# chg60/phamclust

Measured on AMD Instinct MI355X. Metric: genome-pairs/sec, higher is better.
Workload: dtype int32; 1 GPU; synth(5000,5000) -m peq: full N x N distance-matrix fill; `value` = fills with the genomes resident in HBM and the matrix left in HBM (upload and D2H excluded: see value_wall); n_genomes=5000, n_phams=5000, metric_selector=peq, genome_pairs=12497500, n_genes=531832, n_residues=111773410, parallelism=static pair shard over 1 GPU(s)

## Files before the change

### phamclust_amd/csrc/pc_align.hip

```cpp
#include <numeric>

#include "pc_host.h"

static int small_launch_min() {
    static const int v = [] { const char* e = getenv("PC_SMALL_LAUNCH_MIN"); const int x = e ? atoi(e) : 0; return x > 0 ? x : 192; }();
    return v;
}
static int run_align_classes(pc_ctx* c, const PcTask* task_list, const uint32_t* task_begin , const int32_t* cls_max_lb,
                             uint2* res, hipStream_t st, pc_stats* stats, int ppos) {
    const int nbase = c->ncls_all;
    struct Launch { uint32_t begin, end; int base, mode, max_lb; };
    std::vector<Launch> launches;
    for (int b = 0; b < nbase; ++b) {
        const uint32_t* tb = task_begin + (size_t)b * PC_WAVE_MODES;
        if (tb[PC_WAVE_MODES] == tb[0]) continue;
        const uint32_t n0 = tb[1] - tb[0], n1 = tb[2] - tb[1], n2 = tb[3] - tb[2];
        const int bv = pc_class_variant(b);
        const uint32_t least = (bv >= 0 && pc_nw_variant_w(bv) >= 32) ? 1u : (uint32_t)small_launch_min();
        const bool own2 = n2 >= least, own1 = n1 + (own2 ? 0u : n2) >= least;
        uint32_t at = tb[0];
        const int max_lb = cls_max_lb[b * PC_WAVE_MODES];
        auto put = [&](uint32_t n, int mode) { if (n) launches.push_back({at, at + n, b, mode, max_lb}); at += n; };
        if (own1) { put(n0, PC_MODE_CLASS); put(n1 + (own2 ? 0u : n2), n1 ? PC_MODE_TWO_WAVES : PC_MODE_ONE_WAVE); }
        else put(n0 + n1 + (own2 ? 0u : n2), n0 ? PC_MODE_CLASS : n1 ? PC_MODE_TWO_WAVES : PC_MODE_ONE_WAVE);
// ... 544 lines not shown
        local.n_chunks = 1;
        *stats = local;
    }
    return PC_OK;
}

extern "C" int pc_reduce_dev(pc_ctx* c, int metric, int as_distance, const void* res_dev, void* out_condensed_dev, void* stream) {
    if (!c || !c->uploaded || !c->plan.valid) { pc_set_error("pc_reduce_dev: pc_plan_dev first"); return PC_ERR_STATE; }
    if (!c->plan.whole) { pc_set_error("pc_reduce_dev: the plan in the context is not a whole-matrix plan of an unsharded context (pc_plan_dev)"); return PC_ERR_STATE; }
    if (metric == PC_AAI_PPOS) metric = PC_AAI;
    if (metric != PC_AAI && metric != PC_PEQ) { pc_set_error("pc_reduce_dev: metric %d", metric); return PC_ERR_ARG; }
    if (!out_condensed_dev || (!res_dev && c->plan.n_distinct > 0)) { pc_set_error("pc_reduce_dev: NULL argument"); return PC_ERR_ARG; }
    PC_ON_DEVICE(c);
    hipStream_t st = (hipStream_t)stream;
    int rc = wait_last_work(c, st, true); if (rc != PC_OK) return rc;
    rc = stage_reduce(c, metric, as_distance, (const uint2*)res_dev, (double*)out_condensed_dev, st);
    int rc2 = mark_work(c, st);
    return rc != PC_OK ? abi_rc(rc) : rc2;
}

extern "C" int pc_align_pairs(pc_ctx* c, const int32_t* a_gene, const int32_t* b_gene, int64_t n, int variant,
                              int32_t* n_ident, int32_t* n_diag) {
    if (!c || !c->uploaded) { pc_set_error("pc_align_pairs: upload first"); return PC_ERR_STATE; }
    if (n < 0 || (n > 0 && (!a_gene || !b_gene || !n_ident || !n_diag))) { pc_set_error("pc_align_pairs: NULL argument"); return PC_ERR_ARG; }
    if (n == 0) return PC_OK;
    if (n >= 0x7fffffffLL) { pc_set_error("pc_align_pairs: too many pairs"); return PC_ERR_LIMIT; }
    if (!c->residues_ready) { pc_set_error("pc_align_pairs: the residues are not on the device (pc_upload_residues)"); return PC_ERR_STATE; }
    PC_ON_DEVICE(c);
    int rc = wait_last_work(c, nullptr, false); if (rc != PC_OK) return rc;
    c->plan.valid = false;
    const int G = c->dev.G;
    const int nvar = pc_nw_num_variants();
    int forced = -2;
    if (variant < 0) forced = -1;
    else if (variant > 0) {
        for (int v = 0; v < nvar; ++v) if (pc_nw_variant_w(v) == variant) forced = v;
        if (forced == -2) { pc_set_error("pc_align_pairs: no systolic variant with %d columns per lane", variant); return PC_ERR_ARG; }
    }
    std::vector<int> cls(n);
    std::vector<int32_t> sums(n);
    for (int64_t k = 0; k < n; ++k) {
        if (a_gene[k] < 0 || a_gene[k] >= G || b_gene[k] < 0 || b_gene[k] >= G) { pc_set_error("pc_align_pairs: gene index out of range at %lld", (long long)k); return PC_ERR_ARG; }
        const int la = c->h_gene_len[a_gene[k]], lb = c->h_gene_len[b_gene[k]];
        if (la == 0 || lb == 0) { pc_set_error("pc_align_pairs: empty translation at %lld", (long long)k); return PC_ERR_DATA; }
        int v = forced == -2 ? pc_nw_choose_variant(lb) : forced;
        if (v >= 0 && lb > 64 * pc_nw_variant_w(v) && pc_nw_variant_w(v) < 32) { pc_set_error("pc_align_pairs: column gene of %d residues does not fit variant w=%d (strip-mined passes exist for w = 32, 48, 64)", lb, pc_nw_variant_w(v)); return PC_ERR_ARG; }
        cls[k] = pc_class_of(lb, v, c->h_gene_odd[b_gene[k]] != 0);
        sums[k] = la + lb;
    }
    std::vector<int64_t> order(n);
    std::iota(order.begin(), order.end(), 0);
    std::sort(order.begin(), order.end(), [&](int64_t x, int64_t y) {
        if (cls[x] != cls[y]) return cls[x] < cls[y];
        if (b_gene[x] != b_gene[y]) return b_gene[x] < b_gene[y];
        return x < y;
    });
    std::vector<int32_t> rows(n); std::vector<uint32_t> dest(n); std::vector<PcTask> tasks;
    const int nlc = pc_num_classes() * PC_WAVE_MODES;
    std::vector<uint32_t> cls_task_begin(nlc + 1, 0);
    std::vector<int> cls_maxlb(nlc, 0);
    {
        for (int64_t i = 0; i < n;) {
            const int64_t k = order[i];
            int64_t j = i;
            while (j < n && cls[order[j]] == cls[k] && b_gene[order[j]] == b_gene[k]) ++j;
            const int lb = c->h_gene_len[b_gene[k]];
            const bool odd = c->h_gene_odd[b_gene[k]] != 0;
            const PcBucketCut cut = pc_bucket_cut(lb, j - i, cls[k], odd, forced == -2);
            const int per = cut.per, rem_cls = cut.rem_base;
            const int64_t jmain = i + cut.n_main;
            auto put = [&](int64_t r0, int64_t r1, int base) {
                PcTask t; t.gene = b_gene[k]; t.begin = (int32_t)r0; t.end = (int32_t)r1;
                t.pad = pc_task_launch_class(lb, (int)(r1 - r0), base, forced == -2);
                cls_maxlb[t.pad] = std::max(cls_maxlb[t.pad], lb);
                tasks.push_back(t);
            };
            for (int64_t r = i; r < jmain; r += per) put(r, std::min<int64_t>(jmain, r + per), cls[k]);
            if (rem_cls >= 0) put(jmain, j, rem_cls);
            for (int64_t r = i; r < j; ++r) { rows[r] = a_gene[order[r]]; dest[r] = (uint32_t)order[r]; }
            i = j;
        }
        std::stable_sort(tasks.begin(), tasks.end(), [&](const PcTask& x, const PcTask& y) {
            if (x.pad != y.pad) return x.pad < y.pad;
            const int64_t wx = (int64_t)(x.end - x.begin) * c->h_gene_len[x.gene], wy = (int64_t)(y.end - y.begin) * c->h_gene_len[y.gene];
            return wx > wy;
        });
        size_t at = 0;
        for (int lc = 0; lc <= nlc; ++lc) { while (at < tasks.size() && tasks[at].pad < lc) ++at; cls_task_begin[lc] = (uint32_t)at; }
    }
    DevBuf d_sums, d_ident, d_diag;
    hipStream_t st = c->stream;
    if ((rc = upload_vec(c->b_bucket_row, rows)) || (rc = upload_vec(c->b_bucket_dest, dest)) || (rc = upload_vec(c->b_tasks, tasks)) ||
        (rc = c->b_res.ensure(n * 8)) || (rc = upload_vec(d_sums, sums)) || (rc = d_ident.ensure(n * 4)) || (rc = d_diag.ensure(n * 4))) return abi_rc(rc);
    (void)hipEventRecord(c->ev[1], st);
    for (int lc = 0; lc < nlc; ++lc) {
        const int nt = (int)(cls_task_begin[lc + 1] - cls_task_begin[lc]);
        if (nt <= 0) continue;
        void* scratch = nullptr; size_t sbytes = 0;
        const int base = lc / PC_WAVE_MODES, v = pc_class_variant(base);
        if (v < 0 || pc_launch_is_strip(v, cls_maxlb[lc], lc % PC_WAVE_MODES, 0)) {
            sbytes = v < 0 ? pc_nw_fallback_scratch_bytes(cls_maxlb[lc]) : pc_nw_strip_scratch_bytes(c->max_gene_len, c->n_cu);
            if ((rc = c->b_scratch.ensure(sbytes))) return abi_rc(rc);
            scratch = c->b_scratch.p; sbytes = c->b_scratch.cap;
        }
        rc = pc_launch_nw(v, c->dev, c->b_tasks.as<PcTask>() + cls_task_begin[lc], nt, c->b_bucket_row.as<int32_t>(),
                          c->b_bucket_dest.as<uint32_t>(), c->b_res.as<uint2>(), scratch, sbytes, cls_maxlb[lc], 0, c->tie_rule, pc_class_compare_only(base), st,
// ... 15 lines not shown
```

### phamclust_amd/csrc/pc_nw.hip

```cpp
#include "pc_nw_systolic.h"


struct PcCell { int Ho, E, F; uint32_t SH, SE, SF; };

__device__ __forceinline__ PcCell pc_cell(int Hol, int El, uint32_t SHl, uint32_t SEl, int Hou, int Fu, uint32_t SHu,
                                          uint32_t SFu, int Hod, uint32_t SHd, int sp, bool eq, int rule) {
    PcCell c;
    const int Ee = El - PC_EXT, Fe = Fu - PC_EXT;
    c.E = max(Hol, Ee);
    c.SE = ((rule & 2) ? Hol >= Ee : Hol > Ee) ? SHl : SEl;
    c.F = max(Hou, Fe);
    c.SF = ((rule & 4) ? Hou >= Fe : Hou > Fe) ? SHu : SFu;
    const int D = Hod + sp;
    const int H = max(max(D, c.E), c.F);
    const uint32_t SD = SHd + 0x10000u + (eq ? 1u : 0u);
    const uint32_t ST = (rule & 1) ? ((H == c.E) ? c.SE : c.SF) : ((H == c.F) ? c.SF : c.SE);
    c.SH = (H == D) ? SD : ST;
    c.Ho = H - PC_OPEN;
    return c;
}

__global__ __launch_bounds__(64) void k_nw_general(PcDev d, const PcTask* __restrict__ tasks, int ntasks,
                                                   const int32_t* __restrict__ bucket_row,
                                                   const uint32_t* __restrict__ bucket_dest, uint2* __restrict__ res,
                                                   int4* __restrict__ scratch, int64_t scratch_stride, int ppos, int rule) {
    __shared__ int8_t tab[24][24];
    for (int i = threadIdx.x; i < 576; i += 64) tab[i / 24][i % 24] = (int8_t)(c_b62[i / 24][i % 24] + PC_OPEN);
    __syncthreads();
    int4* sc = scratch + (int64_t)blockIdx.x * scratch_stride;
    const int lane = threadIdx.x;
    for (int task = blockIdx.x; task < ntasks; task += gridDim.x) {
        const PcTask tk = tasks[task];
        const int lb = d.gene_len[tk.gene];
// ... 48 lines not shown

static const int g_variant_w[] = {2, 3, 4, 5, 6, 7, 8, 9, 10, 11, 12, 13, 14, 15, 16, 17, 18, 19, 20, 22, 24, 32, 48, 64};
static const int g_num_variants = (int)(sizeof(g_variant_w) / sizeof(int));

static bool class_inc16(int W, int G);
int pc_nw_num_variants() { return g_num_variants; }
int pc_nw_variant_w(int v) { return (v >= 0 && v < g_num_variants) ? g_variant_w[v] : 0; }
int pc_nw_variant_takes_any_byte(int v) { return v < 0 || v >= g_num_variants || g_variant_w[v] > PC_INC16_MAX_W; }

static bool strip_enabled() { static const bool off = getenv("PC_STRIP") && !atoi(getenv("PC_STRIP")); return !off; }
int pc_nw_launch_is_strip(int variant, int max_lb, int wave_mode, int ppos) {
    if (variant < 0 || variant >= g_num_variants) return 0;
    const int W = g_variant_w[variant];
    if (max_lb > 64 * W) return 1;
    return (!ppos && W >= 32 && wave_mode != PC_MODE_CLASS && strip_enabled()) ? 1 : 0;
}
int pc_nw_strip_passes(int lb, int variant) {
    if (variant < 0 || variant >= g_num_variants || lb <= 0) return 0;
    const int cols = 64 * g_variant_w[variant];
    return (lb + cols - 1) / cols;
}
static int choose_strip_variant(int lb) {
    if (!strip_enabled()) return -1;
    int best = -1; double best_cost = 0;
    for (int v = 0; v < g_num_variants; ++v) {
        const int W = g_variant_w[v];
        if (W < 32) continue;
        const double pen = W >= 64 ? 1.15 : W >= 48 ? 1.08 : 1.04;
        const double cost = (double)pc_nw_strip_passes(lb, v) * (W + 1.0) * pen;
        if (best < 0 || cost < best_cost) { best = v; best_cost = cost; }
    }
    return best;
}
int pc_nw_choose_variant(int lb) {
    if (lb <= 0) return -1;
    if (lb > 64 * PC_MAX_W) return choose_strip_variant(lb);
    int best = -1; double best_cost = 0;
    for (int v = 0; v < g_num_variants; ++v) {
        const int W = g_variant_w[v];
        const int G = (lb + W - 1) / W;
        if (G > 64) continue;
        int nseg = 64 / G; if (nseg > 16) nseg = 16;
        const double pen = W >= 64 ? 1.15 : W >= 48 ? 1.08 : W >= 32 ? 1.04 : W >= 24 ? 1.022 : (W >= 22 ? 1.014 : 1.0);
        constexpr double c0 = 0.3, c1 = 0.535;
        constexpr double cell = 0.94;
        const double cost = (W + c0 + c1 * nseg) * pen * (class_inc16(W, G) ? cell : 1.0) / nseg;
        if (best < 0 || cost < best_cost) { best = v; best_cost = cost; }
    }
    return best;
}

int pc_nw_choose_remainder(int lb, int r, int main_variant) {
    static const bool off = getenv("PC_REMAINDER") && !strcmp(getenv("PC_REMAINDER"), "0");
    if (off || lb <= 0 || r <= 0 || main_variant < 0 || main_variant >= g_num_variants) return -1;
    constexpr double c0 = 0.3, c1 = 0.535;
    auto step_cost = [&](int v, int& nseg) {
        const int W = g_variant_w[v], G = (lb + W - 1) / W;
        if (G > 64) { nseg = 0; return 0.0; }
        nseg = 64 / G; if (nseg > PC_MAX_SEG) nseg = PC_MAX_SEG;
        const double pen = W >= 64 ? 1.15 : W >= 48 ? 1.08 : W >= 32 ? 1.04 : W >= 24 ? 1.022 : (W >= 22 ? 1.014 : 1.0);
        return (W + c0 + c1 * nseg) * pen;
    };
    int nseg0; const double stay = step_cost(main_variant, nseg0);
    if (nseg0 <= 1 || r >= nseg0) return -1;
    constexpr double margin = 0.7;
    int best = -1; double best_cost = margin * stay;
    for (int v = 0; v < g_num_variants; ++v) {
        int nseg; const double sc = step_cost(v, nseg);
        if (!nseg) continue;
        const double cost = sc * ((r + nseg - 1) / nseg);
        if (cost < best_cost) { best = v; best_cost = cost; }
    }
    return best;
}

static size_t systolic_lds_bytes(int W, int G, int nw, bool inc16, bool any_bucket = false) {
    const int Gb = pc_nw_g_bucket(G), rpl = 64 / Gb;
    int nseg_max = (Gb == 8 || any_bucket) ? PC_MAX_SEG : 64 / (Gb / 2 + 1); if (nseg_max > PC_MAX_SEG) nseg_max = PC_MAX_SEG;
    const size_t lines = (inc16 && Gb == 64) ? (size_t)2 * ((pc_prof_rows(inc16) + 1) / 2)
                                             : (size_t)((pc_prof_rows(inc16) + rpl - 1) / rpl);
    return (size_t)(144 + nw * pc_wave_lds_dwords(nseg_max)) * 4 + lines * pc_prof_row_dwords(W, inc16) * 256;
}
int pc_nw_g_bucket(int G) { return G <= 8 ? 8 : (G <= 16 ? 16 : (G <= 32 ? 32 : 64)); }
static bool class_inc16(int W, int G) {
    static const int force = getenv("PC_INC16") ? atoi(getenv("PC_INC16")) : -1;
    if (W > PC_INC16_MAX_W) return false;
    const int Gb = pc_nw_g_bucket(G);
    if (Gb > 32) return false;
    if (force >= 0) return force != 0;
    return (Gb <= 16 && W <= 22) || (Gb == 32 && W >= 11 && W <= 19);
}
static bool mode_inc16(int W, int G, int cell_mode) {
    if (cell_mode == 2) return W <= PC_INC16_MAX_W && G <= 64;
    return cell_mode == 0 && class_inc16(W, G);
}
static int waves_for(int W, int G, int cell_mode) {
    const int Gb = pc_nw_g_bucket(G), top = pc_max_waves(W);
    const bool inc16 = mode_inc16(W, G, cell_mode);
    if (!inc16) return PC_MIN_WAVES;
    for (int nw = PC_MIN_WAVES; nw <= top; nw *= 2)
        if ((int)((size_t)160 * 1024 / systolic_lds_bytes(W, Gb, nw, inc16)) * nw >= 16) return nw;
    return top;
}
int pc_nw_class_waves(int variant, int lb, int compare_only) {
    if (variant < 0 || variant >= g_num_variants || lb <= 0) return PC_MIN_WAVES;
    const int W = g_variant_w[variant];
    return waves_for(W, (lb + W - 1) / W, compare_only != 0 ? 1 : 0);
}
#define PC_STRIP_PPOS_MAX_LB 8191
int pc_nw_ppos_systolic(int variant, int max_lb) {
    if (variant < 0 || variant >= g_num_variants || max_lb <= 0) return 0;
    const int W = g_variant_w[variant];
    if (max_lb > 64 * W) return (W == PC_INC16_MAX_W && strip_enabled() && max_lb <= PC_STRIP_PPOS_MAX_LB) ? 1 : 0;
    return mode_inc16(W, (max_lb + W - 1) / W, 2) ? 1 : 0;
}
int pc_nw_ppos_variant(int max_lb) {
    for (int v = g_num_variants - 1; v >= 0; --v) if (pc_nw_ppos_systolic(v, max_lb)) return v;
    return -1;
}

static int task_budget() {
    static int b = 0;
    if (!b) { const char* e = getenv("PC_TASK_BUDGET"); b = e ? atoi(e) : 0; if (b <= 0) b = PC_TASK_BUDGET; }
    return b;
}
int pc_nw_task_rows(int lb, int variant, int compare_only) {
    if (variant < 0 || variant >= g_num_variants || lb <= 0) return 64;
    const int W = g_variant_w[variant];
    const int G = (lb + W - 1) / W;
    if (G > 64) return PC_STRIP_WAVES;
    int nseg = G > 64 ? 1 : 64 / G; if (nseg > PC_MAX_SEG) nseg = PC_MAX_SEG;
    const int64_t steps = task_budget() / (W + 1);
    int64_t per_stream = steps / (lb + 1); if (per_stream < 1) per_stream = 1;
    const int nw = pc_nw_class_waves(variant, lb, compare_only);
    int64_t rows = per_stream * nw * nseg;
// ... 210 lines not shown
```

### phamclust_amd/hip.py

```python

import ctypes
import os
import weakref

import numpy as np

_variant = os.environ.get("PHAMCLUST_NATIVE_VARIANT", "")
LIB_PATH = os.path.join(os.path.dirname(os.path.abspath(__file__)), "csrc",
                        f"libphamclust_hip_{_variant}.so" if _variant not in ("", "asan") else "libphamclust_hip.so")
METRIC_IDS = {"gcs": 0, "jc": 1, "pocp": 2, "af": 3, "aai": 4, "peq": 5, "aai_ppos": 6}

_u8p = ctypes.POINTER(ctypes.c_uint8)
_i32p = ctypes.POINTER(ctypes.c_int32)
_i64p = ctypes.POINTER(ctypes.c_int64)
_u64p = ctypes.POINTER(ctypes.c_uint64)
_f64p = ctypes.POINTER(ctypes.c_double)


class HipLibraryError(RuntimeError):
    """The HIP library is missing, or one of its entry points returned an error."""


class PcPacked(ctypes.Structure):
    _fields_ = [("n_genomes", ctypes.c_int32), ("n_phams", ctypes.c_int32),
# ... 460 lines not shown
        self._check(self._lib.pc_fill_dev(self._h, METRIC_IDS[metric], int(bool(as_distance)), ctypes.c_void_p(out_ptr),
                                          ctypes.c_void_p(stream or 0), ctypes.byref(stats) if want_stats else None))
        return stats.as_dict() if want_stats else None

    def fill_shard_dev(self, metric, as_distance, shard_ptr, stream=None, want_stats=True):
        stats = PcStats()
        if metric in NEEDS_RESIDUES:
            self.ensure_residues()
        self._check(self._lib.pc_fill_shard_dev(self._h, METRIC_IDS[metric], int(bool(as_distance)),
                                                ctypes.c_void_p(shard_ptr), ctypes.c_void_p(stream or 0),
                                                ctypes.byref(stats) if want_stats else None))
        return stats.as_dict() if want_stats else None

    def assemble_dev(self, gathered_ptr, world, out_ptr, stream=None):
        self._check(self._lib.pc_assemble_dev(self._h, ctypes.c_void_p(gathered_ptr), int(world),
                                              ctypes.c_void_p(out_ptr), ctypes.c_void_p(stream or 0)))

    def plan_dev(self, metric, stream=None):
        stats = PcStats()
        self.ensure_residues()
        self._check(self._lib.pc_plan_dev(self._h, METRIC_IDS[metric], ctypes.c_void_p(stream or 0), ctypes.byref(stats)))
        return stats.as_dict()

    def align_slice_dev(self, slice_rank, slice_world, res_ptr, stream=None, want_stats=True):
        stats = PcStats()
        self._check(self._lib.pc_align_slice_dev(self._h, int(slice_rank), int(slice_world), ctypes.c_void_p(res_ptr),
                                                 ctypes.c_void_p(stream or 0), ctypes.byref(stats) if want_stats else None))
        return stats.as_dict() if want_stats else None

    def reduce_dev(self, metric, as_distance, res_ptr, out_ptr, stream=None):
        self._check(self._lib.pc_reduce_dev(self._h, METRIC_IDS[metric], int(bool(as_distance)), ctypes.c_void_p(res_ptr),
                                            ctypes.c_void_p(out_ptr), ctypes.c_void_p(stream or 0)))

    def align_pairs(self, a_gene, b_gene, variant=0):
        self.ensure_residues()
        a = np.ascontiguousarray(a_gene, dtype=np.int32)
        b = np.ascontiguousarray(b_gene, dtype=np.int32)
        n = a.shape[0]
        ident, diag = np.zeros(n, np.int32), np.zeros(n, np.int32)
        self._check(self._lib.pc_align_pairs(self._h, _ptr(a, _i32p), _ptr(b, _i32p), n, int(variant),
                                             _ptr(ident, _i32p), _ptr(diag, _i32p)))
        return ident, diag

    def set_tie_rule(self, rule):
        self._check(self._lib.pc_set_tie_rule(self._h, int(rule)))

    def tie_rule(self):
        return int(self._lib.pc_get_tie_rule(self._h))

    @staticmethod
    def variant_width(lb):
        return int(load().pc_variant_width(int(lb)))

    @staticmethod
    def task_shape(lb, width=0):
        out = np.zeros(4, dtype=np.int32)
        if load().pc_task_shape(int(lb), int(width), _ptr(out, _i32p)) != 0:
            raise HipLibraryError(load().pc_last_error().decode())
        return dict(zip(("rows", "waves", "streams", "passes"), out.tolist()))

    @staticmethod
    def ppos_width(max_lb):
        return int(load().pc_ppos_width(int(max_lb)))

    WAVE_MODES = 3

    @staticmethod
# ... 174 lines not shown
```

Before: 24.85 million genome-pairs/s.

## Choose systolic variant and inc16 cell mode from measured rate table

Adds a table of measured per-step costs for each systolic width, segment bucket and cell mode. Variant choice, remainder-variant choice and the inc16 decision now use it, switching away from the analytic model only when the table gap exceeds the noise spread, and skipping pinned length ranges. Variant choice is memoised per column length, and a like_fill flag lets align_pairs reproduce the fill's bucketing with a forced variant. The table is tied to one device and build, so it may choose badly if kernels or hardware change.

Result: faster. 25.34 million genome-pairs/s, median of 6 (+2.0%).

```diff
diff --git a/phamclust_amd/csrc/pc_align.hip b/phamclust_amd/csrc/pc_align.hip
--- a/phamclust_amd/csrc/pc_align.hip
+++ b/phamclust_amd/csrc/pc_align.hip
@@ -600,6 +600,8 @@
     const int G = c->dev.G;
     const int nvar = pc_nw_num_variants();
     int forced = -2;
+    const bool like_fill = variant >= 1000;
+    if (like_fill) variant -= 1000;
     if (variant < 0) forced = -1;
     else if (variant > 0) {
         for (int v = 0; v < nvar; ++v) if (pc_nw_variant_w(v) == variant) forced = v;
@@ -634,12 +636,12 @@
             while (j < n && cls[order[j]] == cls[k] && b_gene[order[j]] == b_gene[k]) ++j;
             const int lb = c->h_gene_len[b_gene[k]];
             const bool odd = c->h_gene_odd[b_gene[k]] != 0;
-            const PcBucketCut cut = pc_bucket_cut(lb, j - i, cls[k], odd, forced == -2);
+            const PcBucketCut cut = pc_bucket_cut(lb, j - i, cls[k], odd, forced == -2 || like_fill);
             const int per = cut.per, rem_cls = cut.rem_base;
             const int64_t jmain = i + cut.n_main;
             auto put = [&](int64_t r0, int64_t r1, int base) {
                 PcTask t; t.gene = b_gene[k]; t.begin = (int32_t)r0; t.end = (int32_t)r1;
-                t.pad = pc_task_launch_class(lb, (int)(r1 - r0), base, forced == -2);
+                t.pad = pc_task_launch_class(lb, (int)(r1 - r0), base, forced == -2 || like_fill);
                 cls_maxlb[t.pad] = std::max(cls_maxlb[t.pad], lb);
                 tasks.push_back(t);
             };
diff --git a/phamclust_amd/csrc/pc_nw.hip b/phamclust_amd/csrc/pc_nw.hip
--- a/phamclust_amd/csrc/pc_nw.hip
+++ b/phamclust_amd/csrc/pc_nw.hip
@@ -1,4 +1,7 @@
 #include "pc_nw_systolic.h"
+#include "pc_nw_rates.h"
+#include <algorithm>
+#include <vector>
 
 
 struct PcCell { int Ho, E, F; uint32_t SH, SE, SF; };
@@ -113,46 +116,139 @@
     }
     return best;
 }
-int pc_nw_choose_variant(int lb) {
-    if (lb <= 0) return -1;
-    if (lb > 64 * PC_MAX_W) return choose_strip_variant(lb);
+static double model_step(int W, int nseg) {
+    const double pen = W >= 64 ? 1.15 : W >= 48 ? 1.08 : W >= 32 ? 1.04 : W >= 24 ? 1.022 : (W >= 22 ? 1.014 : 1.0);
+    return (W + 0.3 + 0.535 * nseg) * pen;
+}
+static int inc16_forced() { static const int force = getenv("PC_INC16") ? atoi(getenv("PC_INC16")) : -1; return force; }
+static bool model_inc16(int W, int Gb) {
+    if (W > PC_INC16_MAX_W || Gb > 32) return false;
+    if (inc16_forced() >= 0) return inc16_forced() != 0;
+    return (Gb <= 16 && W <= 22) || (Gb == 32 && W >= 11 && W <= 19);
+}
+static int nseg_of(int G) { const int n = 64 / G; return n > PC_MAX_SEG ? PC_MAX_SEG : n; }
+static int model_choose_variant(int lb) {
     int best = -1; double best_cost = 0;
     for (int v = 0; v < g_num_variants; ++v) {
         const int W = g_variant_w[v];
         const int G = (lb + W - 1) / W;
         if (G > 64) continue;
-        int nseg = 64 / G; if (nseg > 16) nseg = 16;
-        const double pen = W >= 64 ? 1.15 : W >= 48 ? 1.08 : W >= 32 ? 1.04 : W >= 24 ? 1.022 : (W >= 22 ? 1.014 : 1.0);
-        constexpr double c0 = 0.3, c1 = 0.535;
-        constexpr double cell = 0.94;
-        const double cost = (W + c0 + c1 * nseg) * pen * (class_inc16(W, G) ? cell : 1.0) / nseg;
+        const int nseg = nseg_of(G);
+        const bool inc16 = model_inc16(W, pc_nw_g_bucket(G));
+        const double cost = model_step(W, nseg) * (inc16 ? 0.94 : 1.0) / nseg;
         if (best < 0 || cost < best_cost) { best = v; best_cost = cost; }
     }
     return best;
+}
+
+static bool rate_at(int W, int G, int cell, double& step, double& spread) {
+    const int Gb = pc_nw_g_bucket(G);
+    const PcRatePoint *lo = nullptr, *hi = nullptr;
+    for (int i = 0; i < pc_nw_n_rates; ++i) {
+        const PcRatePoint& p = pc_nw_rates[i];
+        if (p.W != W || p.cell != cell || pc_nw_g_bucket(p.G) != Gb) continue;
+        if (p.G <= G && (!lo || p.G > lo->G)) lo = &p;
+        if (p.G >= G && (!hi || p.G < hi->G)) hi = &p;
+    }
+    if (lo && hi) {
+        const double t = hi->G == lo->G ? 0.0 : (double)(G - lo->G) / (hi->G - lo->G);
+        step = lo->step + t * (hi->step - lo->step);
+        spread = std::max(lo->spread, hi->spread);
+        return true;
+    }
+    const PcRatePoint* p = lo ? lo : hi;
+    if (!p || nseg_of(p->G) != nseg_of(G)) return false;
+    step = p->step; spread = p->spread;
+    return true;
+}
+static int rate_table_use() { static const int m = getenv("PC_RATE_TABLE") ? atoi(getenv("PC_RATE_TABLE")) : 3; return m; }
+static bool rate_pinned(int lb) {
+    if (!(rate_table_use() & 1)) return true;
+    for (int i = 0; i < pc_nw_n_rate_pins; ++i) if (lb >= pc_nw_rate_pins[i][0] && lb <= pc_nw_rate_pins[i][1]) return true;
+    return false;
+}
+static bool inc16_fits(int W, int Gb);
+static bool rate_of(int v, int lb, double& cost, double& spread) {
+    const int W = g_variant_w[v], G = (lb + W - 1) / W;
+    if (G > 64) return false;
+    double s, e;
+    if (!rate_at(W, G, class_inc16(W, G) ? 1 : 0, s, e)) return false;
+    cost = s / nseg_of(G); spread = e / nseg_of(G);
+    return true;
+}
+static int choose_max_w() { static const int w = getenv("PC_CHOOSE_MAX_W") ? atoi(getenv("PC_CHOOSE_MAX_W")) : 0; return w; }
+static int choose_variant_uncached(int lb) {
+    int best = model_choose_variant(lb);
+    const int cap = choose_max_w();
+    if (cap > 0 && best >= 0 && g_variant_w[best] > cap && lb <= 64 * cap) {
+        best = -1; double best_cost = 0;
+        for (int v = 0; v < g_num_variants; ++v) {
+            const int W = g_variant_w[v], G = (lb + W - 1) / W;
+            if (G > 64 || W > cap) continue;
+            const double cost = model_step(W, nseg_of(G)) / nseg_of(G);
+            if (best < 0 || cost < best_cost) { best = v; best_cost = cost; }
+        }
+        return best;
+    }
+    double c0, e0;
+    if (best < 0 || rate_pinned(lb) || !rate_of(best, lb, c0, e0)) return best;
+    double best_cost = c0;
+    for (int v = 0; v < g_num_variants; ++v) {
+        double c, e;
+        if (!rate_of(v, lb, c, e)) continue;
+        if (c + e + e0 < c0 && c < best_cost) { best = v; best_cost = c; }
+    }
+    return best;
+}
+int pc_nw_choose_variant(int lb) {
+    if (lb <= 0) return -1;
+    if (lb > 64 * PC_MAX_W) return choose_strip_variant(lb);
+    static const std::vector<int8_t> memo = [] {
+        std::vector<int8_t> m(64 * PC_MAX_W + 1, -1);
+        for (int l = 1; l <= 64 * PC_MAX_W; ++l) m[l] = (int8_t)choose_variant_uncached(l);
+        return m;
+    }();
+    return memo[lb];
 }
 
 int pc_nw_choose_remainder(int lb, int r, int main_variant) {
     static const bool off = getenv("PC_REMAINDER") && !strcmp(getenv("PC_REMAINDER"), "0");
     if (off || lb <= 0 || r <= 0 || main_variant < 0 || main_variant >= g_num_variants) return -1;
-    constexpr double c0 = 0.3, c1 = 0.535;
-    auto step_cost = [&](int v, int& nseg) {
-        const int W = g_variant_w[v], G = (lb + W - 1) / W;
-        if (G > 64) { nseg = 0; return 0.0; }
-        nseg = 64 / G; if (nseg > PC_MAX_SEG) nseg = PC_MAX_SEG;
-        const double pen = W >= 64 ? 1.15 : W >= 48 ? 1.08 : W >= 32 ? 1.04 : W >= 24 ? 1.022 : (W >= 22 ? 1.014 : 1.0);
-        return (W + c0 + c1 * nseg) * pen;
-    };
-    int nseg0; const double stay = step_cost(main_variant, nseg0);
+    const int W0 = g_variant_w[main_variant], G0 = (lb + W0 - 1) / W0;
+    if (G0 > 64) return -1;
+    const int nseg0 = nseg_of(G0);
     if (nseg0 <= 1 || r >= nseg0) return -1;
     constexpr double margin = 0.7;
-    int best = -1; double best_cost = margin * stay;
+    int best = -1; double best_cost = margin * model_step(W0, nseg0);
     for (int v = 0; v < g_num_variants; ++v) {
-        int nseg; const double sc = step_cost(v, nseg);
-        if (!nseg) continue;
-        const double cost = sc * ((r + nseg - 1) / nseg);
+        const int W = g_variant_w[v], G = (lb + W - 1) / W;
+        if (G > 64) continue;
+        const int nseg = nseg_of(G);
+        const double cost = model_step(W, nseg) * ((r + nseg - 1) / nseg);
         if (cost < best_cost) { best = v; best_cost = cost; }
     }
-    return best;
+    double s0, e0;
+    if (rate_pinned(lb) || !rate_at(W0, G0, 0, s0, e0)) return best;
+    auto tab = [&](int v, double& c, double& e) {
+        const int W = g_variant_w[v], G = (lb + W - 1) / W;
+        if (G > 64 || !rate_at(W, G, 0, c, e)) return false;
+        const int rounds = (r + nseg_of(G) - 1) / nseg_of(G);
+        c *= rounds; e *= rounds;
+        return true;
+    };
+    double cur = margin * s0, cur_e = margin * e0;
+    if (best >= 0) {
+        double c, e;
+        if (!tab(best, c, e)) return best;
+        if (c - e > cur + cur_e) best = -1; else { cur = c; cur_e = e; }
+    }
+    int pick = best; double pick_cost = cur;
+    for (int v = 0; v < g_num_variants; ++v) {
+        double c, e;
+        if (v == main_variant || !tab(v, c, e)) continue;
+        if (c + e + cur_e < cur && c < pick_cost) { pick = v; pick_cost = c; }
+    }
+    return pick;
 }
 
 static size_t systolic_lds_bytes(int W, int G, int nw, bool inc16, bool any_bucket = false) {
@@ -164,12 +260,34 @@
 }
 int pc_nw_g_bucket(int G) { return G <= 8 ? 8 : (G <= 16 ? 16 : (G <= 32 ? 32 : 64)); }
 static bool class_inc16(int W, int G) {
-    static const int force = getenv("PC_INC16") ? atoi(getenv("PC_INC16")) : -1;
+    const int force = inc16_forced();
     if (W > PC_INC16_MAX_W) return false;
     const int Gb = pc_nw_g_bucket(G);
+    if (force == 2) return inc16_fits(W, Gb);
     if (Gb > 32) return false;
     if (force >= 0) return force != 0;
-    return (Gb <= 16 && W <= 22) || (Gb == 32 && W >= 11 && W <= 19);
+    static const std::vector<int8_t> by_table = [] {
+        std::vector<int8_t> t((PC_INC16_MAX_W + 1) * 4, -1);
+        for (int w = 1; w <= PC_INC16_MAX_W; ++w)
+            for (int b = 0; b < 3; ++b) {
+                const int gb = 8 << b;
+                if (!inc16_fits(w, gb) || !(rate_table_use() & 2)) continue;
+                double prof = 0, comp = 0, err = 0; int n = 0;
+                for (int i = 0; i < pc_nw_n_rates; ++i) {
+                    const PcRatePoint& p = pc_nw_rates[i];
+                    if (p.W != w || p.cell != 1 || pc_nw_g_bucket(p.G) != gb) continue;
+                    for (int k = 0; k < pc_nw_n_rates; ++k) {
+                        const PcRatePoint& q = pc_nw_rates[k];
+                        if (q.W == w && q.cell == 0 && q.G == p.G) { prof += p.step; comp += q.step; err += p.spread + q.spread; ++n; }
+                    }
+                }
+                if (n && prof + err < comp) t[w * 4 + b] = 1;
+                if (n && comp + err < prof) t[w * 4 + b] = 0;
+            }
+        return t;
+    }();
+    const int said = by_table[W * 4 + (Gb == 8 ? 0 : Gb == 16 ? 1 : 2)];
+    return said >= 0 ? said != 0 : model_inc16(W, Gb);
 }
 static bool mode_inc16(int W, int G, int cell_mode) {
     if (cell_mode == 2) return W <= PC_INC16_MAX_W && G <= 64;
@@ -182,6 +300,12 @@
     for (int nw = PC_MIN_WAVES; nw <= top; nw *= 2)
         if ((int)((size_t)160 * 1024 / systolic_lds_bytes(W, Gb, nw, inc16)) * nw >= 16) return nw;
     return top;
+}
+static bool inc16_fits(int W, int Gb) {
+    if (W > PC_INC16_MAX_W) return false;
+    for (int nw = PC_MIN_WAVES; nw <= pc_max_waves(W); nw *= 2)
+        if ((int)((size_t)160 * 1024 / systolic_lds_bytes(W, Gb, nw, true)) * nw >= 16) return true;
+    return false;
 }
 int pc_nw_class_waves(int variant, int lb, int compare_only) {
     if (variant < 0 || variant >= g_num_variants || lb <= 0) return PC_MIN_WAVES;
diff --git a/phamclust_amd/csrc/pc_nw_rates.h b/phamclust_amd/csrc/pc_nw_rates.h
--- /dev/null
+++ b/phamclust_amd/csrc/pc_nw_rates.h
@@ -0,0 +1,409 @@
+#pragma once
+#include <stdint.h>
+
+struct PcRatePoint { uint8_t W, cell, G; float step, spread; };
+static constexpr PcRatePoint pc_nw_rates[] = {
+    {3, 0, 20, 5.0269f, 0.0074f},
+    {3, 0, 60, 3.9152f, 0.0304f},
+    {3, 1, 20, 4.7997f, 0.0026f},
+    {3, 1, 60, 3.8189f, 0.0149f},
+    {4, 0, 15, 5.9179f, 0.0062f},
+    {4, 0, 30, 5.2726f, 0.0340f},
+    {4, 0, 60, 4.7408f, 0.0096f},
+    {4, 1, 15, 5.6104f, 0.0118f},
+    {4, 1, 30, 5.0525f, 0.0274f},
+    {4, 1, 60, 4.5723f, 0.0265f},
+    {5, 0, 12, 7.7296f, 0.0077f},
+    {5, 0, 20, 6.9422f, 0.0142f},
+    {5, 0, 30, 6.2327f, 0.0040f},
+    {5, 0, 32, 6.1804f, 0.0132f},
+    {5, 0, 60, 5.6183f, 0.0239f},
+    {5, 1, 12, 7.3177f, 0.0014f},
+    {5, 1, 20, 6.6924f, 0.0173f},
+    {5, 1, 30, 6.0127f, 0.0211f},
+    {5, 1, 32, 5.9562f, 0.0197f},
+    {5, 1, 60, 5.7193f, 0.0323f},
+    {6, 0, 10, 9.2533f, 0.0047f},
+    {6, 0, 20, 7.8994f, 0.0298f},
+    {6, 0, 29, 7.2003f, 0.0277f},
+    {6, 0, 30, 7.1101f, 0.0580f},
+    {6, 0, 57, 6.4509f, 0.0111f},
+    {6, 1, 10, 8.8597f, 0.0063f},
+    {6, 1, 20, 7.6008f, 0.0284f},
+    {6, 1, 29, 6.8571f, 0.0255f},
+    {6, 1, 30, 6.7887f, 0.0334f},
+    {6, 1, 57, 6.5386f, 0.0346f},
+    {7, 0, 9, 11.0309f, 0.0130f},
+    {7, 0, 15, 8.9389f, 0.0209f},
+    {7, 0, 20, 8.8723f, 0.0211f},
+    {7, 0, 29, 8.1011f, 0.0222f},
+    {7, 0, 32, 7.9627f, 0.0173f},
+    {7, 0, 58, 7.0196f, 0.0498f},
+    {7, 1, 9, 10.4481f, 0.0119f},
+    {7, 1, 15, 8.4222f, 0.0629f},
+    {7, 1, 20, 8.5124f, 0.0267f},
+    {7, 1, 29, 7.7157f, 0.0279f},
+    {7, 1, 32, 7.6141f, 0.0122f},
+    {7, 1, 58, 6.9111f, 0.0134f},
+    {8, 0, 8, 11.4049f, 0.0220f},
+    {8, 0, 13, 9.9965f, 0.0528f},
+    {8, 0, 15, 10.0954f, 0.0082f},
+    {8, 0, 19, 9.8710f, 0.0459f},
+    {8, 0, 20, 9.8467f, 0.0329f},
+    {8, 0, 30, 8.9061f, 0.0696f},
+    {8, 0, 63, 7.9228f, 0.0518f},
+    {8, 1, 8, 10.7049f, 0.0038f},
+    {8, 1, 13, 9.4514f, 0.0386f},
+    {8, 1, 15, 9.5168f, 0.0137f},
+    {8, 1, 19, 9.4644f, 0.0420f},
+    {8, 1, 20, 9.3941f, 0.0112f},
+    {8, 1, 30, 8.4546f, 0.0367f},
+    {8, 1, 63, 7.5904f, 0.0076f},
+    {9, 0, 7, 14.4320f, 0.0046f},
+    {9, 0, 12, 12.1778f, 0.0295f},
+    {9, 0, 14, 11.2717f, 0.0771f},
+    {9, 0, 16, 10.9413f, 0.0240f},
+    {9, 0, 19, 11.0529f, 0.0454f},
+    {9, 0, 20, 10.9090f, 0.0377f},
+    {9, 0, 29, 9.8611f, 0.0846f},
+    {9, 1, 7, 13.8454f, 0.0119f},
+    {9, 1, 12, 11.7246f, 0.0375f},
+    {9, 1, 14, 10.7684f, 0.0532f},
+    {9, 1, 16, 10.3545f, 0.0244f},
+    {9, 1, 19, 11.1768f, 0.0031f},
+    {9, 1, 20, 11.0276f, 0.0225f},
+    {9, 1, 29, 9.7754f, 0.0197f},
+    {10, 0, 6, 16.7173f, 0.0359f},
+    {10, 0, 10, 13.9202f, 0.0247f},
+    {10, 0, 12, 13.5514f, 0.0230f},
+    {10, 0, 14, 12.3543f, 0.0485f},
+    {10, 0, 15, 12.3571f, 0.0241f},
+    {10, 0, 16, 12.2544f, 0.0557f},
+    {10, 0, 20, 12.1937f, 0.0480f},
+    {10, 0, 30, 11.1374f, 0.0281f},
+    {10, 0, 60, 10.2533f, 0.0253f},
+    {10, 1, 6, 15.6581f, 0.0237f},
+    {10, 1, 10, 12.9743f, 0.0544f},
+    {10, 1, 12, 12.5531f, 0.0071f},
+    {10, 1, 14, 11.4541f, 0.0251f},
+    {10, 1, 15, 11.4668f, 0.0578f},
+    {10, 1, 16, 11.2780f, 0.0141f},
+    {10, 1, 20, 11.8619f, 0.0151f},
+    {10, 1, 30, 10.4659f, 0.0154f},
+    {10, 1, 60, 10.1072f, 0.0541f},
+    {11, 0, 6, 17.9345f, 0.0404f},
+    {11, 0, 10, 14.9950f, 0.0370f},
+    {11, 0, 11, 14.6766f, 0.0422f},
+    {11, 0, 14, 13.4144f, 0.0571f},
+    {11, 0, 15, 13.3390f, 0.0455f},
+    {11, 0, 16, 13.2736f, 0.0263f},
+    {11, 0, 19, 13.1480f, 0.0276f},
+    {11, 0, 20, 12.8812f, 0.0303f},
+    {11, 0, 28, 11.9839f, 0.0364f},
+    {11, 0, 31, 11.8134f, 0.1520f},
+    {11, 0, 64, 11.2704f, 0.0414f},
+    {11, 1, 6, 16.8223f, 0.0244f},
+    {11, 1, 10, 14.0123f, 0.0148f},
+    {11, 1, 11, 13.6633f, 0.0502f},
+    {11, 1, 14, 12.5163f, 0.0076f},
+    {11, 1, 15, 12.3400f, 0.0428f},
+    {11, 1, 16, 12.2704f, 0.0188f},
+    {11, 1, 19, 12.8611f, 0.0389f},
+    {11, 1, 20, 12.6738f, 0.0296f},
+    {11, 1, 28, 11.4061f, 0.0523f},
+    {11, 1, 31, 11.2786f, 0.0840f},
+    {11, 1, 64, 11.0799f, 0.0444f},
+    {12, 0, 5, 19.5960f, 0.0600f},
+    {12, 0, 9, 17.0537f, 0.0292f},
+    {12, 0, 10, 16.2071f, 0.0209f},
+    {12, 0, 12, 15.4884f, 0.0480f},
+    {12, 0, 14, 14.4388f, 0.0465f},
+    {12, 0, 15, 14.3443f, 0.0680f},
+    {12, 0, 19, 13.8783f, 0.0390f},
+    {12, 0, 20, 14.0021f, 0.0510f},
+    {12, 0, 29, 12.7323f, 0.0865f},
+    {12, 0, 59, 12.1733f, 0.0504f},
+    {12, 1, 5, 18.2086f, 0.0055f},
+    {12, 1, 9, 15.7592f, 0.0862f},
+    {12, 1, 10, 15.0709f, 0.0237f},
+    {12, 1, 12, 14.3177f, 0.0886f},
+    {12, 1, 14, 13.3077f, 0.0384f},
+    {12, 1, 15, 13.2404f, 0.0500f},
+    {12, 1, 19, 13.5966f, 0.0438f},
+    {12, 1, 20, 13.5538f, 0.0574f},
+    {12, 1, 29, 12.1208f, 0.0143f},
+    {12, 1, 59, 11.9651f, 0.0195f},
+    {13, 0, 5, 21.4020f, 0.0277f},
+    {13, 0, 8, 17.1268f, 0.0329f},
+    {13, 0, 10, 17.3885f, 0.0495f},
+    {13, 0, 11, 16.6940f, 0.0260f},
+    {13, 0, 12, 16.7601f, 0.0323f},
+    {13, 0, 14, 15.3517f, 0.1314f},
+    {13, 0, 16, 15.0589f, 0.0823f},
+    {13, 0, 19, 15.1492f, 0.0546f},
+    {13, 0, 20, 15.1695f, 0.0338f},
+    {13, 0, 27, 13.6790f, 0.0595f},
+    {13, 0, 31, 13.4248f, 0.0392f},
+    {13, 0, 54, 13.0628f, 0.0838f},
+    {13, 0, 62, 13.1378f, 0.0206f},
+    {13, 1, 5, 20.4191f, 0.0349f},
+    {13, 1, 8, 16.2970f, 0.0447f},
+    {13, 1, 10, 16.7466f, 0.0705f},
+    {13, 1, 11, 16.0521f, 0.1117f},
+    {13, 1, 12, 16.1055f, 0.0723f},
+    {13, 1, 14, 14.6925f, 0.0653f},
+    {13, 1, 16, 14.4792f, 0.0481f},
+    {13, 1, 19, 15.0362f, 0.0450f},
+    {13, 1, 20, 14.8944f, 0.0461f},
+    {13, 1, 27, 13.8744f, 0.0485f},
+    {13, 1, 31, 13.3244f, 0.0047f},
+    {14, 0, 5, 23.2257f, 0.0650f},
+    {14, 0, 8, 18.7467f, 0.0273f},
+    {14, 0, 9, 20.0282f, 0.0697f},
+    {14, 0, 10, 18.6729f, 0.0298f},
+    {14, 0, 11, 18.3028f, 0.0328f},
+    {14, 0, 12, 18.3323f, 0.0246f},
+    {14, 0, 13, 16.6494f, 0.1105f},
+    {14, 0, 15, 16.4852f, 0.0390f},
+    {14, 0, 16, 16.1225f, 0.0185f},
+    {14, 0, 19, 16.5082f, 0.0377f},
+    {14, 0, 29, 14.8729f, 0.1207f},
+    {14, 0, 58, 14.5225f, 0.0321f},
+    {14, 1, 5, 21.4801f, 0.0163f},
+    {14, 1, 8, 17.2517f, 0.0244f},
+    {14, 1, 9, 18.6754f, 0.0454f},
+    {14, 1, 10, 17.4126f, 0.0281f},
+    {14, 1, 11, 17.1789f, 0.0434f},
+    {14, 1, 12, 17.0699f, 0.0578f},
+    {14, 1, 13, 15.6060f, 0.0991f},
+    {14, 1, 15, 15.5126f, 0.0268f},
+    {14, 1, 16, 15.0514f, 0.1368f},
+    {14, 1, 19, 15.6456f, 0.0627f},
+    {14, 1, 29, 14.1495f, 0.0201f},
+    {15, 0, 4, 23.2376f, 0.0629f},
+    {15, 0, 7, 21.7056f, 0.0168f},
+    {15, 0, 8, 19.7947f, 0.0764f},
+    {15, 0, 10, 19.6174f, 0.1022f},
+    {15, 0, 11, 18.3389f, 0.0523f},
+    {15, 0, 12, 19.2315f, 0.2056f},
+    {15, 0, 14, 17.4756f, 0.0430f},
+    {15, 0, 15, 17.2351f, 0.0819f},
+    {15, 0, 16, 17.3505f, 0.0217f},
+    {15, 0, 18, 17.4839f, 0.0350f},
+    {15, 0, 20, 17.4043f, 0.0311f},
+    {15, 0, 27, 15.6409f, 0.0320f},
+    {15, 0, 54, 15.5033f, 0.0097f},
+    {15, 1, 4, 21.5653f, 0.0068f},
+    {15, 1, 7, 20.2433f, 0.0530f},
+    {15, 1, 8, 18.3749f, 0.0545f},
+    {15, 1, 10, 18.4188f, 0.1058f},
+    {15, 1, 11, 17.1703f, 0.0309f},
+    {15, 1, 12, 18.0837f, 0.0859f},
+    {15, 1, 14, 16.4847f, 0.0670f},
+    {15, 1, 15, 16.1753f, 0.1161f},
+    {15, 1, 16, 16.1297f, 0.0307f},
+    {15, 1, 18, 17.1287f, 0.0134f},
+    {15, 1, 20, 16.5569f, 0.0171f},
+    {15, 1, 27, 15.3456f, 0.0183f},
+    {16, 0, 4, 24.4414f, 0.0174f},
+    {16, 0, 7, 22.8599f, 0.0032f},
+    {16, 0, 8, 20.8301f, 0.0379f},
+    {16, 0, 9, 22.0554f, 0.0391f},
+    {16, 0, 10, 20.6548f, 0.0710f},
+    {16, 0, 11, 20.5278f, 0.0340f},
+    {16, 0, 12, 20.1179f, 0.0061f},
+    {16, 0, 13, 18.5058f, 0.0702f},
+    {16, 0, 14, 18.1973f, 0.0485f},
+    {16, 0, 15, 18.3490f, 0.0292f},
+    {16, 0, 19, 18.4405f, 0.0413f},
+    {16, 0, 32, 16.5184f, 0.1003f},
+    {16, 0, 63, 16.8364f, 0.0165f},
+    {16, 1, 4, 22.5830f, 0.0387f},
+    {16, 1, 7, 21.2773f, 0.1517f},
+    {16, 1, 8, 19.4222f, 0.1032f},
+    {16, 1, 9, 20.5498f, 0.0651f},
+    {16, 1, 10, 19.3480f, 0.1072f},
+    {16, 1, 11, 19.1096f, 0.0840f},
+    {16, 1, 12, 18.9929f, 0.0960f},
+    {16, 1, 13, 17.3077f, 0.1059f},
+    {16, 1, 14, 17.0574f, 0.1685f},
+    {16, 1, 15, 17.0941f, 0.0188f},
+    {16, 1, 19, 17.4149f, 0.0639f},
+    {16, 1, 32, 15.4716f, 0.0370f},
+    {17, 0, 4, 25.8639f, 0.0206f},
+    {17, 0, 6, 25.2919f, 0.1672f},
+    {17, 0, 8, 22.0120f, 0.0172f},
+    {17, 0, 9, 23.2139f, 0.1123f},
+    {17, 0, 10, 21.9488f, 0.0399f},
+    {17, 0, 11, 21.2819f, 0.0126f},
+    {17, 0, 12, 21.2220f, 0.0938f},
+    {17, 0, 13, 19.2794f, 0.0919f},
+    {17, 0, 15, 19.5368f, 0.0374f},
+    {17, 0, 16, 19.1293f, 0.0424f},
+    {17, 0, 18, 19.5424f, 0.0608f},
+    {17, 0, 20, 19.0486f, 0.0287f},
+    {17, 0, 30, 17.5445f, 0.0384f},
+    {17, 0, 59, 17.8469f, 0.0359f},
+    {17, 1, 4, 23.8200f, 0.0573f},
+    {17, 1, 6, 23.3979f, 0.0469f},
+    {17, 1, 8, 20.4515f, 0.0303f},
+    {17, 1, 9, 21.8117f, 0.0307f},
+    {17, 1, 10, 20.4952f, 0.0299f},
+    {17, 1, 11, 20.1726f, 0.1308f},
+    {17, 1, 12, 19.8813f, 0.1064f},
+    {17, 1, 13, 18.2283f, 0.0376f},
+    {17, 1, 15, 18.0352f, 0.0065f},
+    {17, 1, 16, 17.5595f, 0.1300f},
+    {17, 1, 18, 19.3744f, 0.0453f},
+    {17, 1, 20, 18.2543f, 0.1037f},
+    {17, 1, 30, 16.4973f, 0.0517f},
+    {18, 0, 4, 27.1234f, 0.0220f},
+    {18, 0, 6, 26.3898f, 0.0343f},
+    {18, 0, 7, 24.6390f, 0.0446f},
+    {18, 0, 8, 22.6463f, 0.0418f},
+    {18, 0, 9, 24.2116f, 0.0942f},
+    {18, 0, 10, 22.7117f, 0.2380f},
+    {18, 0, 12, 22.1643f, 0.0240f},
+    {18, 0, 14, 20.5196f, 0.0702f},
+    {18, 0, 15, 20.1388f, 0.0828f},
+    {18, 0, 19, 19.8339f, 0.0543f},
+    {18, 0, 28, 18.4287f, 0.0425f},
+    {18, 0, 56, 18.7487f, 0.0128f},
+    {18, 1, 4, 24.8837f, 0.0218f},
+    {18, 1, 6, 24.5011f, 0.0470f},
+    {18, 1, 7, 23.1716f, 0.0492f},
+    {18, 1, 8, 20.8068f, 0.0366f},
+    {18, 1, 9, 22.7960f, 0.0827f},
+    {18, 1, 10, 21.2848f, 0.1120f},
+    {18, 1, 12, 20.8468f, 0.0825f},
+    {18, 1, 14, 18.9437f, 0.0825f},
+    {18, 1, 15, 18.5836f, 0.0596f},
+    {18, 1, 19, 19.0916f, 0.0252f},
+    {18, 1, 28, 17.3258f, 0.1313f},
+    {19, 0, 4, 28.3648f, 0.0290f},
+    {19, 0, 6, 27.5059f, 0.0530f},
+    {19, 0, 7, 25.7542f, 0.0602f},
+    {19, 0, 8, 23.7151f, 0.0650f},
+    {19, 0, 9, 25.3962f, 0.0375f},
+    {19, 0, 10, 23.5225f, 0.0488f},
+    {19, 0, 11, 23.2341f, 0.0519f},
+    {19, 0, 12, 23.0998f, 0.1074f},
+    {19, 0, 14, 21.2194f, 0.1688f},
+    {19, 0, 16, 21.1285f, 0.0724f},
+    {19, 0, 18, 20.7499f, 0.0706f},
+    {19, 0, 27, 19.2774f, 0.0202f},
+    {19, 0, 32, 19.5472f, 0.0707f},
+    {19, 0, 53, 19.6425f, 0.0203f},
+    {19, 0, 64, 19.7736f, 0.0429f},
+    {19, 1, 4, 26.0562f, 0.0243f},
+    {19, 1, 6, 25.5100f, 0.0549f},
+    {19, 1, 7, 24.1583f, 0.0583f},
+    {19, 1, 8, 21.8760f, 0.1631f},
+    {19, 1, 9, 23.9302f, 0.0501f},
+    {19, 1, 10, 22.1798f, 0.0209f},
+    {19, 1, 11, 21.7579f, 0.0516f},
+    {19, 1, 12, 21.5990f, 0.1361f},
+    {19, 1, 14, 19.5827f, 0.0562f},
+    {19, 1, 16, 19.2609f, 0.0883f},
+    {19, 1, 18, 20.7961f, 0.0257f},
+    {19, 1, 27, 18.5794f, 0.1382f},
+    {19, 1, 32, 18.5896f, 0.0521f},
+    {20, 0, 5, 32.7035f, 0.0600f},
+    {20, 0, 6, 30.8903f, 0.0589f},
+    {20, 0, 7, 29.2506f, 0.0236f},
+    {20, 0, 8, 26.2691f, 0.0522f},
+    {20, 0, 9, 29.4807f, 0.4709f},
+    {20, 0, 10, 26.8087f, 0.0502f},
+    {20, 0, 11, 26.7758f, 0.0293f},
+    {20, 0, 12, 26.9267f, 0.0177f},
+    {20, 0, 13, 23.3611f, 0.1163f},
+    {20, 0, 15, 23.4390f, 0.0166f},
+    {20, 0, 20, 23.1405f, 0.0465f},
+    {20, 0, 30, 21.7333f, 0.0231f},
+    {20, 0, 60, 22.9898f, 0.0230f},
+    {20, 1, 5, 31.3617f, 0.0262f},
+    {20, 1, 6, 29.8400f, 0.0710f},
+    {20, 1, 7, 27.7887f, 0.0287f},
+    {20, 1, 8, 24.9470f, 0.0743f},
+    {20, 1, 9, 28.4500f, 0.3336f},
+    {20, 1, 10, 25.6894f, 0.0365f},
+    {20, 1, 11, 25.6913f, 0.0675f},
+    {20, 1, 12, 25.5985f, 0.0220f},
+    {20, 1, 13, 21.7823f, 0.1028f},
+    {20, 1, 15, 22.0029f, 0.0602f},
+    {20, 1, 20, 30.1707f, 0.0156f},
+    {20, 1, 30, 25.9906f, 0.0458f},
+    {22, 0, 5, 34.9929f, 0.0441f},
+    {22, 0, 6, 33.0041f, 0.0609f},
+    {22, 0, 7, 31.0994f, 0.2367f},
+    {22, 0, 8, 28.1120f, 0.1188f},
+    {22, 0, 9, 31.1032f, 0.0793f},
+    {22, 0, 10, 28.5425f, 0.1428f},
+    {22, 0, 11, 26.2270f, 0.0106f},
+    {22, 0, 12, 28.7252f, 0.0684f},
+    {22, 0, 14, 25.1477f, 0.0292f},
+    {22, 0, 16, 24.5797f, 0.0371f},
+    {22, 0, 19, 25.0434f, 0.0118f},
+    {22, 0, 32, 23.9257f, 0.0453f},
+    {22, 0, 55, 24.6428f, 0.0291f},
+    {22, 1, 5, 33.8459f, 0.0679f},
+    {22, 1, 6, 32.3593f, 0.0293f},
+    {22, 1, 7, 29.9848f, 0.2173f},
+    {22, 1, 8, 27.1253f, 0.0402f},
+    {22, 1, 9, 30.5603f, 0.0230f},
+    {22, 1, 10, 27.6922f, 0.1061f},
+    {22, 1, 11, 25.1439f, 0.0463f},
+    {22, 1, 12, 27.2561f, 0.0205f},
+    {22, 1, 14, 23.9169f, 0.1064f},
+    {22, 1, 16, 23.7683f, 0.0521f},
+    {22, 1, 19, 32.9856f, 0.0277f},
+    {22, 1, 32, 28.5735f, 0.0212f},
+    {24, 0, 5, 37.4244f, 0.2100f},
+    {24, 0, 6, 35.4449f, 0.0276f},
+    {24, 0, 7, 33.5470f, 0.0461f},
+    {24, 0, 8, 30.1335f, 0.2173f},
+    {24, 0, 9, 33.4439f, 0.0601f},
+    {24, 0, 10, 31.1389f, 0.0628f},
+    {24, 0, 15, 26.8580f, 0.0272f},
+    {24, 0, 21, 28.2875f, 0.0119f},
+    {24, 0, 30, 26.2676f, 0.0309f},
+    {24, 1, 5, 36.6263f, 0.1065f},
+    {24, 1, 6, 34.0453f, 0.0870f},
+    {24, 1, 7, 32.0867f, 0.1385f},
+    {24, 1, 8, 29.0451f, 0.1947f},
+    {24, 1, 9, 35.7464f, 0.0788f},
+    {24, 1, 10, 34.1012f, 0.0673f},
+    {24, 1, 15, 32.5578f, 0.0342f},
+    {24, 1, 21, 34.0820f, 0.0323f},
+    {24, 1, 30, 31.2363f, 0.0048f},
+    {32, 0, 4, 51.8813f, 0.0295f},
+    {32, 0, 5, 56.5103f, 0.1044f},
+    {32, 0, 7, 50.0625f, 0.1881f},
+    {32, 0, 8, 45.6906f, 0.0925f},
+    {32, 0, 9, 49.3934f, 0.1479f},
+    {32, 0, 16, 41.9517f, 0.0149f},
+    {32, 0, 32, 43.1376f, 0.0279f},
+    {48, 0, 4, 69.3486f, 0.0770f},
+    {48, 0, 9, 71.0540f, 0.2642f},
+    {48, 0, 15, 61.0141f, 0.0673f},
+    {48, 0, 21, 64.8726f, 0.0188f},
+    {64, 0, 16, 124.4441f, 0.7821f},
+    {0, 0, 0, 0.f, 0.f},
+};
+static constexpr int pc_nw_n_rates = (int)(sizeof(pc_nw_rates) / sizeof(pc_nw_rates[0])) - 1;
+static constexpr int pc_nw_rate_pins[][2] = {
+    {57, 60},
+    {105, 105},
+    {106, 108},
+    {127, 128},
+    {129, 133},
+    {137, 140},
+    {154, 154},
+    {161, 162},
+    {177, 180},
+    {193, 198},
+    {273, 273},
+    {289, 294},
+    {0, 0},
+};
+static constexpr int pc_nw_n_rate_pins = (int)(sizeof(pc_nw_rate_pins) / sizeof(pc_nw_rate_pins[0])) - 1;
diff --git a/phamclust_amd/hip.py b/phamclust_amd/hip.py
--- a/phamclust_amd/hip.py
+++ b/phamclust_amd/hip.py
@@ -516,7 +516,9 @@
         self._check(self._lib.pc_reduce_dev(self._h, METRIC_IDS[metric], int(bool(as_distance)), ctypes.c_void_p(res_ptr),
                                             ctypes.c_void_p(out_ptr), ctypes.c_void_p(stream or 0)))
 
-    def align_pairs(self, a_gene, b_gene, variant=0):
+    def align_pairs(self, a_gene, b_gene, variant=0, like_fill=False):
+        if like_fill and variant > 0:
+            variant += 1000
         self.ensure_residues()
         a = np.ascontiguousarray(a_gene, dtype=np.int32)
         b = np.ascontiguousarray(b_gene, dtype=np.int32)
```
